# efirdc/Segmentation-Pipeline

Hardware: AMD Instinct MI355X
Metric: 3D patches/sec (128³, 4ch) train+infer at 1/2/4/8 MI355X; Dice vs CPU ref (higher is better)
Workload: dtype f32 (tensors, results and accumulation; the products of the 3x3x3 convolutions with >= 8 input channels run as six bf16 MFMAs on an EXACT three-way bf16 split of both f32 operands -- error vs f64 equal to the f32 MFMA kernels', profiles/r04_f32x3_accuracy.txt; the same step on v_mfma_f32_32x32x2_f32

## Files before the change

### include/m355seg.h

```cpp
#ifndef M355SEG_H
#define M355SEG_H

#include <stddef.h>
#include <stdint.h>

#ifdef __cplusplus
extern "C" {
#endif

#define M355_ABI_VERSION 3

enum {
  M355_OK = 0,
  M355_EINVALID_ARG = -1,
  M355_EUNSUPPORTED = -2,
  M355_ELAUNCH = -3,
  M355_EWORKSPACE = -4
};

enum { M355_F32 = 0 };

enum { M355_COMPUTE_F32 = 0, M355_COMPUTE_BF16 = 1, M355_COMPUTE_F16 = 2, M355_COMPUTE_F32X3 = 3 };

enum { M355_ACT_NONE = 0, M355_ACT_RELU = 1, M355_ACT_LEAKY_RELU = 2, M355_ACT_ELU = 3, M355_ACT_GELU = 4,
// ... 60 lines not shown
int m355_conv3d_bwd_data_h16(const m355_conv3d_desc* d, const void* dy16, int64_t dy16_batch_stride, const float* w,
                             float* dx, void* workspace, size_t workspace_bytes, void* stream);
size_t m355_conv3d_bwd_weight_h16_workspace(const m355_conv3d_desc* d);
int m355_conv3d_bwd_weight_h16(const m355_conv3d_desc* d, const void* x16, int64_t x16_batch_stride, const void* dy16,
                               int64_t dy16_batch_stride, const float* dy, float* dw, float* dbias, void* workspace,
                               size_t workspace_bytes, void* stream);

int m355_conv3d_plan(const m355_conv3d_desc* d, int32_t which, int32_t* out4);

int m355_conv3d_launch_plan(int32_t entry, const m355_conv3d_desc* d, const int64_t* batch_strides, const uint64_t* pointers,
                            size_t workspace_bytes, int64_t* out12);

size_t m355_conv3d_bwd_data_workspace(const m355_conv3d_desc* d);
int m355_conv3d_bwd_data(const m355_conv3d_desc* d, const float* dy, const float* w,
                         float* dx, void* workspace, size_t workspace_bytes, void* stream);

size_t m355_conv3d_bwd_weight_workspace(const m355_conv3d_desc* d);
int m355_conv3d_bwd_weight(const m355_conv3d_desc* d, const float* x, const float* dy,
                           float* dw, float* dbias,
                           void* workspace, size_t workspace_bytes, void* stream);

size_t m355_conv_transpose3d_workspace(const m355_conv3d_desc* d);
int m355_conv_transpose3d_fwd(const m355_conv3d_desc* d, const float* x, const float* w,
                              const float* bias, float* y,
                              void* workspace, size_t workspace_bytes, void* stream);
int m355_conv_transpose3d_bwd_data(const m355_conv3d_desc* d, const float* dy, const float* w,
                                   float* dx, void* workspace, size_t workspace_bytes,
                                   void* stream);
int m355_conv_transpose3d_bwd_weight(const m355_conv3d_desc* d, const float* x, const float* dy,
                                     float* dw, float* dbias,
                                     void* workspace, size_t workspace_bytes, void* stream);

int m355_conv_transpose3d_plan(const m355_conv3d_desc* d, int32_t which, const void* y_side, int32_t* out4);

int m355_conv_transpose3d_fwd_h16(const m355_conv3d_desc* d, const void* x16, int64_t x16_batch_stride,
                                  const float* w, const float* bias, void* y16, int64_t y16_batch_stride,
                                  int32_t compute, void* stream);

typedef struct m355_norm_desc {
  int32_t N, C;
  int64_t S;
  int32_t groups;
  int32_t act;
  float eps;
  float act_slope;
  int64_t x_batch_stride;
  int64_t y_batch_stride;
  int64_t add_batch_stride;
} m355_norm_desc;

int64_t m355_norm_num_stats(const m355_norm_desc* d);
size_t m355_norm_workspace(const m355_norm_desc* d);

int m355_norm_plan(const m355_norm_desc* d, int32_t which, int32_t* out4);

int m355_norm_stats(const m355_norm_desc* d, const float* x, float* mean, float* rstd,
                    float* running_mean, float* running_var, float momentum,
                    void* workspace, size_t workspace_bytes, void* stream);
int m355_norm_stats_from_partials(const m355_norm_desc* d, const float* stat_partials, int64_t slots,
                                  float* mean, float* rstd, float* running_mean, float* running_var,
                                  float momentum, void* workspace, size_t workspace_bytes, void* stream);
int m355_norm_stats_from_running(const m355_norm_desc* d, const float* running_mean,
                                 const float* running_var, float* mean, float* rstd,
                                 void* stream);
int m355_norm_act_fwd(const m355_norm_desc* d, const float* x, const float* mean,
                      const float* rstd, const float* gamma, const float* beta,
// ... 426 lines not shown
```

### segmentation-pipeline_amd/_lib.py

```python
import ctypes as C
import os

_HERE = os.path.dirname(os.path.abspath(__file__))
LIB_PATH = os.environ.get("M355_LIB_PATH") or os.path.join(_HERE, "libm355seg.so")

M355_OK = 0
ACT_NONE, ACT_RELU, ACT_LEAKY_RELU = 0, 1, 2
ACT_ELU, ACT_GELU, ACT_GELU_TANH, ACT_SILU = 3, 4, 5, 6
COMPUTE_F32, COMPUTE_BF16, COMPUTE_F16, COMPUTE_F32X3 = 0, 1, 2, 3
CONV_W_PACKED, CONV_SOFTMAX, CONV_SIGMOID = 1, 2, 4


class ConvDesc(C.Structure):
    _fields_ = [
        ("N", C.c_int32), ("Cin", C.c_int32), ("Cout", C.c_int32),
        ("D", C.c_int32), ("H", C.c_int32), ("W", C.c_int32),
        ("k", C.c_int32), ("stride", C.c_int32), ("pad", C.c_int32), ("out_pad", C.c_int32),
        ("x_batch_stride", C.c_int64), ("y_batch_stride", C.c_int64),
        ("compute", C.c_int32), ("flags", C.c_int32),
    ]


class PackItem(C.Structure):
    _fields_ = [("desc", ConvDesc), ("which", C.c_int32), ("w", C.c_void_p), ("packed", C.c_void_p)]


class NormDesc(C.Structure):
    _fields_ = [
        ("N", C.c_int32), ("C", C.c_int32), ("S", C.c_int64),
        ("groups", C.c_int32), ("act", C.c_int32),
        ("eps", C.c_float), ("act_slope", C.c_float),
        ("x_batch_stride", C.c_int64), ("y_batch_stride", C.c_int64), ("add_batch_stride", C.c_int64),
    ]


class AugStage(C.Structure):
    _fields_ = [("op", C.c_int32), ("order", C.c_int32), ("a", C.c_float), ("b", C.c_float), ("seed", C.c_uint64),
                ("stats", C.c_void_p), ("vec", C.c_void_p)]

# ... 112 lines not shown
    "m355_act16_pack_scaled": (C.c_int, [_P, _P, _i32, _i32, _i64, _i64, _i64, _i32, _f32, _P]),
    "m355_act16_unpack_scaled": (C.c_int, [_P, _P, _i32, _i32, _i64, _i64, _i64, _i32, _f32, _P]),
    "m355_conv3d_bwd_data_h16_c8": (C.c_int, [_CD, _P, _i64, _P, _P, _i64, _P, _sz, _P]),
    "m355_conv3d_bwd_weight_c8_workspace": (_sz, [_CD]),
    "m355_conv3d_bwd_weight_c8": (C.c_int, [_CD, _P, _i64, _P, _i64, _P, _P, _f32, _P, _sz, _P]),
    "m355_norm_act_bwd_c8": (C.c_int, [_ND, _P, _i64, _P, _i64, _P, _i64, _i32, _i32, _i32, _P, _P, _P, _P, _P, _i64, _P, _P,
                                       C.c_int, _f32, _i32, _P, _sz, _P]),
    "m355_norm_act_bwd_c8_reduce": (C.c_int, [_ND, _P, _i64, _P, _i64, _P, _i64, _i32, _i32, _i32, _P, _P, _P, _P, _P, _P,
                                              C.c_int, _P, _f32, _P, _i32, _P, _sz, _P]),
    "m355_norm_act_bwd_c8_apply": (C.c_int, [_ND, _P, _i64, _P, _i64, _P, _i64, _i32, _i32, _i32, _P, _P, _P, _P, _P, _P, _i64,
                                             _i32, _P]),
    "m355_avgpool3d_2x_bwd_h16": (C.c_int, [_P, _P, _P, _i32, _i32, _i32, _i32, _i32, _i64, _i64, _i64, _i32, _P]),
    "m355_upsample_trilinear2x_fwd_h16": (C.c_int, [_P, _P, _i32, _i32, _i32, _i32, _i32, _i64, _i64, _i32, _P]),
    "m355_upsample_trilinear2x_bwd_h16": (C.c_int, [_P, _P, _i32, _i32, _i32, _i32, _i32, _i64, _i64, _i32, _P]),
    "m355_act16_channel_scale": (C.c_int, [_P, _P, _P, _i32, _i32, _i64, _i64, _i64, _i32, _P]),
    "m355_space_to_depth2_h16": (C.c_int, [_P, _P, _i32, _i32, _i32, _i32, _i32, _i64, _i64, _i32, _P]),
    "m355_depth_to_space2_h16": (C.c_int, [_P, _P, _i32, _i32, _i32, _i32, _i32, _i64, _i64, _i32, _P]),
    "m355_conv_transpose3d_h16_bwd_supported": (_i32, [_CD]),
    "m355_conv_transpose3d_h16_bwd_workspace": (_sz, [_CD]),
    "m355_conv_transpose3d_bwd_data_h16": (C.c_int, [_CD, _P, _i64, _P, _P, _i64, _i32, _P]),
    "m355_conv_transpose3d_bwd_weight_h16": (C.c_int, [_CD, _P, _i64, _P, _i64, _P, _P, _f32, _i32, _P, _sz, _P]),
    "m355_conv3d_plan": (C.c_int, [_CD, _i32, C.POINTER(C.c_int32)]),
    "m355_conv3d_launch_plan": (C.c_int, [_i32, _CD, C.POINTER(_i64), C.POINTER(C.c_uint64), _sz, C.POINTER(_i64)]),
    "m355_conv3d_bwd_data_workspace": (_sz, [_CD]),
    "m355_conv3d_bwd_data": (C.c_int, [_CD, _P, _P, _P, _P, _sz, _P]),
    "m355_conv3d_bwd_weight_workspace": (_sz, [_CD]),
    "m355_conv3d_bwd_weight": (C.c_int, [_CD, _P, _P, _P, _P, _P, _sz, _P]),
    "m355_conv_transpose3d_workspace": (_sz, [_CD]),
    "m355_conv_transpose3d_plan": (C.c_int, [_CD, _i32, _P, C.POINTER(C.c_int32)]),
    "m355_conv_transpose3d_fwd": (C.c_int, [_CD, _P, _P, _P, _P, _P, _sz, _P]),
    "m355_conv_transpose3d_bwd_data": (C.c_int, [_CD, _P, _P, _P, _P, _sz, _P]),
    "m355_conv_transpose3d_bwd_weight": (C.c_int, [_CD, _P, _P, _P, _P, _P, _sz, _P]),
    "m355_conv_transpose3d_fwd_h16": (C.c_int, [_CD, _P, _i64, _P, _P, _P, _i64, _i32, _P]),
    "m355_norm_num_stats": (_i64, [_ND]),
    "m355_norm_workspace": (_sz, [_ND]),
    "m355_norm_plan": (C.c_int, [_ND, _i32, C.POINTER(C.c_int32)]),
    "m355_norm_stats": (C.c_int, [_ND, _P, _P, _P, _P, _P, _f32, _P, _sz, _P]),
    "m355_norm_stats_from_partials": (C.c_int, [_ND, _P, _i64, _P, _P, _P, _P, _f32, _P, _sz, _P]),
    "m355_norm_stats_from_running": (C.c_int, [_ND, _P, _P, _P, _P, _P]),
    "m355_norm_act_fwd": (C.c_int, [_ND, _P, _P, _P, _P, _P, _P, _P, _P]),
    "m355_norm_act_pool_fwd": (C.c_int, [_ND, _P, _P, _P, _P, _P, _P, _P, _i64, _i32, _i32, _i32, _P]),
    "m355_norm_act_bwd": (C.c_int, [_ND, _P, _P, _P, _P, _P, _P, _P, _P, _P, C.c_int, _P, _sz, _P]),
    "m355_norm_act_bwd_pool": (C.c_int, [_ND, _P, _P, _i64, _P, _i64, _i32, _i32, _i32, _P, _P, _P, _P, _P, _P, _P, C.c_int,
                                         _P, _sz, _P]),
    "m355_norm_sums": (C.c_int, [_ND, _P, _P, _i64, _P, _P, _sz, _P]),
    "m355_norm_stats_from_sums": (C.c_int, [_ND, _P, _P, _P, _P, _P, _f32, _P]),
    "m355_norm_act_bwd_reduce": (C.c_int, [_ND, _P, _P, _P, _P, _P, _P, _P, _P, C.c_int, _P, _P, _P, _sz, _P]),
    "m355_norm_act_bwd_apply": (C.c_int, [_ND, _P, _P, _P, _P, _P, _P, _P, _P, _P, _i64, _i32, _P]),
    "m355_norm_act_bwd_h16": (C.c_int, [_ND, _P, _P, _P, _P, _P, _P, _P, _P, _P, C.c_int, _P, _i64, _i32, _P, _sz, _P]),
    "m355_resample_plan": (C.c_int, [_i32, _i32, _i32, _i32, _i32, _i32, C.POINTER(_i64), C.POINTER(C.c_uint64), _i32,
                                     C.POINTER(_i64)]),
    "m355_avgpool3d_2x_fwd": (C.c_int, [_P, _P, _i32, _i32, _i32, _i32, _i32, _i64, _i64, _P]),
    "m355_avgpool3d_2x_bwd": (C.c_int, [_P, _P, _i32, _i32, _i32, _i32, _i32, _i64, _i64, _P]),
    "m355_avgpool3d_2x_bwd_add": (C.c_int, [_P, _P, _P, _i32, _i32, _i32, _i32, _i32, _i64, _i64, _i64, _P]),
    "m355_maxpool3d_2x_fwd": (C.c_int, [_P, _P, _P, _i32, _i32, _i32, _i32, _i32, _i64, _i64, _P]),
    "m355_maxpool3d_2x_bwd": (C.c_int, [_P, _P, _P, _P, _i32, _i32, _i32, _i32, _i32, _i64, _i64, _i64, _P]),
    "m355_maxpool3d_2x_fwd_h16": (C.c_int, [_P, _P, _P, _i32, _i32, _i32, _i32, _i32, _i64, _i64, _i32, _P]),
    "m355_maxpool3d_2x_bwd_h16": (C.c_int, [_P, _P, _P, _P, _i32, _i32, _i32, _i32, _i32, _i64, _i64, _i64, _i32, _P]),
    "m355_upsample_trilinear2x_fwd": (C.c_int, [_P, _P, _i32, _i32, _i32, _i32, _i32, _i64, _i64, _P]),
    "m355_upsample_trilinear2x_bwd": (C.c_int, [_P, _P, _i32, _i32, _i32, _i32, _i32, _i64, _i64, _P]),
    "m355_upsample_nearest2x_fwd": (C.c_int, [_P, _P, _i32, _i32, _i32, _i32, _i32, _i64, _i64, _P]),
    "m355_upsample_nearest2x_bwd": (C.c_int, [_P, _P, _i32, _i32, _i32, _i32, _i32, _i64, _i64, _P]),
    "m355_upsample_trilinear2x_hp_fwd": (C.c_int, [_P, _P, _i32, _i32, _i32, _i32, _i32, _i64, _i64, _P]),
    "m355_upsample_trilinear2x_hp_bwd": (C.c_int, [_P, _P, _i32, _i32, _i32, _i32, _i32, _i64, _i64, _P]),
    "m355_upsample_nearest2x_fwd_h16": (C.c_int, [_P, _P, _i32, _i32, _i32, _i32, _i32, _i64, _i64, _i32, _P]),
    "m355_upsample_nearest2x_bwd_h16": (C.c_int, [_P, _P, _i32, _i32, _i32, _i32, _i32, _i64, _i64, _i32, _P]),
# ... 185 lines not shown
```

### segmentation-pipeline_amd/csrc/abi.cpp

```cpp
#include "common.hpp"
#include <map>
#include <mutex>
#include <tuple>
#include <utility>

namespace m355 {
static thread_local char g_err[512] = "";
void set_error(const char* fmt, ...) {
  va_list ap;
  va_start(ap, fmt);
  vsnprintf(g_err, sizeof(g_err), fmt, ap);
  va_end(ap);
}

static int env_int(const char* name, int dflt) {
  const char* v = getenv(name);
  if (!v || !*v) return dflt;
  return atoi(v);
}
static Tuning read_tuning() {
  Tuning t;
  t.conv_ntw = env_int("M355_CONV_NTW", 0);
  t.conv_ksplit = env_int("M355_CONV_KSPLIT", 0);
  t.conv_slots = env_int("M355_CONV_SLOTS", 0);
  t.conv_persistent = env_int("M355_CONV_PERSISTENT", 1);
  t.no_small = env_int("M355_NO_SMALL", 0);
  t.smallcout_valu = env_int("M355_SMALLCOUT_VALU", 1);
  t.f32x3 = env_int("M355_F32X3", 1);
  t.f32x3_bww = env_int("M355_F32X3_BWW", 1);
  t.f32x3_edge = env_int("M355_F32X3_EDGE", 0);
  t.f32x3_convt = env_int("M355_F32X3_CONVT", 1);
  t.bww_nsplit = env_int("M355_BWW_NSPLIT", 0);
  t.bww_gen = env_int("M355_BWW_GEN", 2);
  t.bww_queue = env_int("M355_BWW_QUEUE", 1);
  t.h16_persistent = env_int("M355_H16_PERSISTENT", 1);
  t.tile16 = env_int("M355_TILE16", 1);
  t.convt_h16 = env_int("M355_CONVT_H16", 1);
  t.h16_w8 = env_int("M355_H16_W8", 1);
  t.h16_oneshot = env_int("M355_H16_ONESHOT", 1);
  t.h16_xcd = env_int("M355_H16_XCD", 1);
  t.conv_cube = env_int("M355_CONV_CUBE", 3);
  t.h16_order = env_int("M355_H16_ORDER", 3);
  t.fuse_softmax = env_int("M355_FUSE_SOFTMAX", 1);
  t.convt_wgs = env_int("M355_CONVT_WGS", 0);
  t.h16_stagger = env_int("M355_H16_STAGGER", 2);
  return t;
}
static Tuning g_tuning = read_tuning();
const Tuning& tuning() { return g_tuning; }

int num_cus() {
  static int cache[64] = {0};
  int dev = 0;
  if (hipGetDevice(&dev) != hipSuccess || dev < 0 || dev >= 64) {
    (void)hipGetLastError();
    return 256;
  }
  if (cache[dev] == 0) {
    int n = 0;
    if (hipDeviceGetAttribute(&n, hipDeviceAttributeMultiprocessorCount, dev) != hipSuccess || n <= 0) {
      (void)hipGetLastError();
      n = 256;
    }
    cache[dev] = n;
// ... 86 lines not shown
```

### segmentation-pipeline_amd/csrc/common.hpp

```cpp
#pragma once
#include <hip/hip_runtime.h>
#include <stdint.h>
#include <stdio.h>
#include <stdarg.h>
#include <stdlib.h>
#include <algorithm>
#include "../../include/m355seg.h"

namespace m355 {

void set_error(const char* fmt, ...);

static inline int64_t ceil_div(int64_t a, int64_t b) { return (a + b - 1) / b; }
static inline int64_t round_up(int64_t a, int64_t b) { return ceil_div(a, b) * b; }

static inline int check_launch(const char* what) {
  hipError_t e = hipGetLastError();
  if (e != hipSuccess) {
    set_error("%s: launch failed: %s", what, hipGetErrorString(e));
    return M355_ELAUNCH;
  }
  return M355_OK;
}

// ... 13 lines not shown
template <typename T>
__device__ __forceinline__ T wave_sum(T v) {
#pragma unroll
  for (int off = 32; off > 0; off >>= 1) v += __shfl_xor(v, off, 64);
  return v;
}

template <typename T, int NT, bool BCAST = false>
__device__ __forceinline__ T block_sum(T v, T* scratch) {
  v = wave_sum(v);
  const int lane = threadIdx.x & 63, w = threadIdx.x >> 6;
  __syncthreads();
  if (lane == 0) scratch[w] = v;
  __syncthreads();
  T r = T(0);
  if (BCAST || threadIdx.x == 0) {
#pragma unroll
    for (int i = 0; i < NT / 64; ++i) r += scratch[i];
  }
  return r;
}

__device__ __forceinline__ float sigmoid_f32(float v) { return 1.f / (1.f + expf(-v)); }

struct Tuning {
  int conv_ntw = 0, conv_ksplit = 0, conv_slots = 0, conv_persistent = 1;
  int no_small = 0, smallcout_valu = 1, bww_nsplit = 0, bww_gen = 2, bww_queue = 1, h16_persistent = 1, tile16 = 1, convt_h16 = 1, h16_w8 = 1, h16_oneshot = 1, h16_xcd = 1;
  int conv_cube = 3, h16_order = 3;
  int fuse_softmax = 1;
  int f32x3 = 1;
  int f32x3_bww = 1;
  int f32x3_edge = 0;
  int f32x3_convt = 1;
  int convt_wgs = 0;
  int h16_stagger = 2;
};
const Tuning& tuning();

static inline int64_t dense_or(int64_t stride, int64_t dense) { return stride ? stride : dense; }

int num_cus();

int* queue_state(hipStream_t st);
int* overflow_flag();

}
```

### segmentation-pipeline_amd/csrc/conv3d_common.hpp

```cpp
#pragma once
#include "common.hpp"
#include "h16.hpp"
#include "conv3d_route.hpp"

namespace m355 {


__device__ __forceinline__ int opaque(int v) {
  asm volatile("" : "+v"(v));
  return v;
}

__device__ __forceinline__ void queue_leave(int* __restrict__ counter) {
  if (threadIdx.x == 0) {
    if (atomicAdd(counter + 8, 1) == (int)gridDim.x - 1) {
#pragma unroll
      for (int r = 0; r < 9; ++r) counter[r] = 0;
    }
  }
}

template <int NTW, int GX>
struct FwdTile {
  static constexpr int GY = 32 / GX;
// ... 120 lines not shown
          s1[r] += t;
          s2[r] = fmaf(t, t, s2[r]);
        }
      }
      if (ok) {
#pragma unroll
        for (int r = 0; r < 4; ++r)
          if (ob + r < Cout) dst[base + (int64_t)r * DHW] = v[r];
      }
    }
  if (stat) {
#pragma unroll
    for (int r = 0; r < 4; ++r) {
#pragma unroll
      for (int off = 8; off >= 1; off >>= 1) {
        s1[r] += __shfl_xor(s1[r], off, 64);
        s2[r] += __shfl_xor(s2[r], off, 64);
      }
    }
    if ((lane & 15) == 0) {
#pragma unroll
      for (int r = 0; r < 4; ++r)
        if (ob + r < Cout) {
          stat[(int64_t)(ob + r) * 2] = s1[r];
          stat[(int64_t)(ob + r) * 2 + 1] = s2[r];
        }
    }
  }
}

int convt_fwd_x3_nvt(int Cin);
void launch_convt_fwd_x3(int nvt, dim3 grid, const float* x, const float* w, const float* bias, float* y, int Cin, int Cout,
                         int D, int H, int W, int64_t xbs, int64_t ybs, int mt_per_wg, hipStream_t st);

enum class ConvtKind {
  Direct,
  MfmaF32,
  X3,
  C8,
  H16,
  Unsupported
};
struct ConvtRoute {
  ConvtKind kind;
  int nvt;
  int mt;
  int mt_per_wg;
  int ks_n, ng;
  dim3 grid;
  size_t lds;
  int split, o_per_split;
  size_t slab_bytes;
  size_t dbias_offset, dbias_bytes;
  size_t workspace_bytes;
  int32_t plan_code[4];
};
ConvtRoute route_convt(const m355_conv3d_desc* d, int which, bool y_side_ok);
ConvtRoute route_convt_c8(const m355_conv3d_desc* d, int which);

struct ConvCall {
  const m355_conv3d_desc* d;
  const float* in;
  const void* in16;
  const float* w;
  const float* bias;
  const float* add;
// ... 86 lines not shown
```

### segmentation-pipeline_amd/csrc/conv3d_f32x3.hip

```cpp
#include "conv3d_common.hpp"

namespace m355 {

typedef __bf16 bf16x8 __attribute__((ext_vector_type(8)));
typedef unsigned u32x4 __attribute__((ext_vector_type(4)));

constexpr int X3_PAIRS = 14;
constexpr int X3_QUADS = 7;
__host__ __device__ constexpr int x3_pair_tap(int pair, int half) {
  return pair < 9 ? pair * 3 + half : (pair < 12 ? (pair - 9) * 9 + half * 3 + 2 : (pair == 12 ? half * 9 + 8 : 26));
}

__device__ __forceinline__ void x3_split(float v, unsigned& hi, unsigned& mid, unsigned& lo) {
  const unsigned u = __float_as_uint(v);
  hi = u & 0xffff0000u;
  const float r1 = (u & 0x7f800000u) == 0x7f800000u ? 0.f : v - __uint_as_float(hi);
  mid = __float_as_uint(r1) & 0xffff0000u;
  lo = __float_as_uint(r1 - __uint_as_float(mid));
}
__device__ __forceinline__ unsigned x3_pack(unsigned a, unsigned b) { return __builtin_amdgcn_perm(b, a, 0x07060302u); }

__device__ __forceinline__ void pack_w3_x3_item(const float* __restrict__ w, u32x4* __restrict__ wq, int64_t i, int Cout_w,
                                                int Cin_w, int kin, int mout, int nchunks, int transpose) {
  const int lane = (int)(i & 63);
// ... 1052 lines not shown
#pragma unroll
      for (int g = 0; g < NG; ++g) {
        if (v0 + g * 32 + l32 >= S) continue;
#pragma unroll
        for (int b = 0; b < 2; ++b)
          *reinterpret_cast<float2*>(yo + obase[g] + (int64_t)b * OW) =
              make_float2(acc[g][q * 4 + b * 2] + bv, acc[g][q * 4 + b * 2 + 1] + bv);
      }
    }
    mt += 4;
  }
}

int convt_fwd_x3_nvt(int Cin) {
  const int64_t cin2 = round_up(Cin, 16);
  for (int nvt : {128, 64, 32})
    if (cin2 * nvt * 6 <= 65536) return nvt;
  return 0;
}

void launch_convt_fwd_x3(int nvt, dim3 grid, const float* x, const float* w, const float* bias, float* y, int Cin, int Cout,
                         int D, int H, int W, int64_t xbs, int64_t ybs, int mt_per_wg, hipStream_t st) {
  const size_t lds = (size_t)round_up(Cin, 16) * nvt * 6;
#define M355_CONVT_X3(NVT) \
  hipLaunchKernelGGL(convt_k2s2_fwd_x3_kernel<NVT>, grid, dim3(256), lds, st, x, w, bias, y, Cin, Cout, D, H, W, xbs, ybs, mt_per_wg)
  switch (nvt) {
    case 128: M355_CONVT_X3(128); break;
    case 64: M355_CONVT_X3(64); break;
    default: M355_CONVT_X3(32); break;
  }
#undef M355_CONVT_X3
}

}
```

### segmentation-pipeline_amd/csrc/convt.hip

```cpp
#include "conv3d_common.hpp"

namespace m355 {

typedef float f32x16 __attribute__((ext_vector_type(16)));


template <int NVT>
__global__ __launch_bounds__(256) void convt_k2s2_fwd_mfma_kernel(
    const float* __restrict__ x, const float* __restrict__ w, const float* __restrict__ bias,
    float* __restrict__ y, int Cin, int Cout, int D, int H, int W, int64_t xbs, int64_t ybs, int mt_per_wg) {
  extern __shared__ float xs[];
  constexpr int NG = NVT / 32, P = 256 / NVT;
  const int tid = threadIdx.x, lane = tid & 63;
  const int wave = __builtin_amdgcn_readfirstlane(tid >> 6);
  const int half = lane >> 5, l32 = lane & 31;
  const int S = D * H * W;
  const int v0 = blockIdx.x * NVT;
  const int n = blockIdx.z;
  const float* xn = x + (int64_t)n * xbs;
  float* yn = y + (int64_t)n * ybs;
  constexpr int KC = 8;
  const int Cin2 = (Cin + 2 * KC - 1) / (2 * KC) * (2 * KC);
  const int OH = 2 * H, OW = 2 * W;
  const int64_t OS = (int64_t)S * 8;
// ... 1184 lines not shown
  if (compute == M355_COMPUTE_BF16) { M355_CONVT_FWD_T(__bf16) } else { M355_CONVT_FWD_T(_Float16) }
#undef M355_CONVT_FWD_T
#undef M355_CONVT_C8
#undef M355_CONVT_H16
}

static void launch_convt_bwd_data_h16(const ConvtRoute& r, const m355_conv3d_desc* d, const void* dy16, int64_t ybs,
                                      const float* w, void* dx16, int64_t xbs, int compute, hipStream_t st) {
  int* oflag = compute == M355_COMPUTE_F16 ? overflow_flag() : nullptr;
#define M355_CTBD(HT, MTW)                                                                                               \
  hipLaunchKernelGGL((convt_k2s2_bwd_data_h16_kernel<HT, MTW>), r.grid, dim3(256), r.lds, st, (const HT*)dy16, w,        \
                     (HT*)dx16, d->Cin, d->Cout, d->D, d->H, d->W, ybs, xbs, r.mt_per_wg, oflag)
#define M355_CTBD_T(HT)                                                  \
  if (r.mt_per_wg == 1) M355_CTBD(HT, 1); else if (r.mt_per_wg == 2) M355_CTBD(HT, 2); else M355_CTBD(HT, 4);
  if (compute == M355_COMPUTE_BF16) { M355_CTBD_T(__bf16) } else { M355_CTBD_T(_Float16) }
#undef M355_CTBD_T
#undef M355_CTBD
}

static void launch_convt_bww_c8(const ConvtRoute& r, const m355_conv3d_desc* d, const void* x16, int64_t xbs, const void* dy16,
                                int64_t ybs, float* dw, float grad_unscale, int compute, float* slab, hipStream_t st) {
#define M355_CTBW(HT, CT)                                                                                                 \
  hipLaunchKernelGGL((convt_k2s2_bww_c8_kernel<HT, CT>), r.grid, dim3(256), 0, st, (const HT*)x16, (const HT*)dy16, slab,  \
                     d->N, d->Cin, d->Cout, d->D, d->H, d->W, xbs, ybs, r.split, (int)r.grid.z)
#define M355_CTBW_T(HT) if (r.mt == 1) M355_CTBW(HT, 1); else if (r.mt == 2) M355_CTBW(HT, 2); else M355_CTBW(HT, 4);
  if (compute == M355_COMPUTE_BF16) { M355_CTBW_T(__bf16) } else { M355_CTBW_T(_Float16) }
#undef M355_CTBW_T
#undef M355_CTBW
  const int64_t total = (int64_t)d->Cin * d->Cout * 8;
  hipLaunchKernelGGL(convt_slab_reduce_t_kernel, dim3((unsigned)ceil_div(total, 64)), dim3(256), 0, st, slab, dw, d->Cin,
                     d->Cout, r.split, grad_unscale, overflow_flag());
}

}

using namespace m355;

extern "C" size_t m355_conv_transpose3d_workspace(const m355_conv3d_desc* d) {
  return d ? std::max(route_convt(d, 2, true).workspace_bytes, route_convt(d, 1, true).workspace_bytes) : 0;
}
extern "C" int32_t m355_conv_transpose3d_h16_bwd_supported(const m355_conv3d_desc* d) {
  return d && route_convt_c8(d, 1).kind != ConvtKind::Unsupported ? 1 : 0;
}
extern "C" size_t m355_conv_transpose3d_h16_bwd_workspace(const m355_conv3d_desc* d) {
  return d ? route_convt_c8(d, 2).workspace_bytes : 0;
}
extern "C" int m355_conv_transpose3d_plan(const m355_conv3d_desc* d, int32_t which, const void* y_side, int32_t* out4) {
  if (int rc = validate_convt(d, "conv_transpose3d_plan")) return rc;
  M355_REQUIRE(out4 && which >= 0 && which <= 5, M355_EINVALID_ARG, "conv_transpose3d_plan: null pointer or which not in 0..5");
  const ConvtRoute r = which < 3 ? route_convt(d, which, convt_y_side_ok(convt_geom(d), y_side)) : route_convt_c8(d, which - 3);
  std::copy_n(r.plan_code, 4, out4);
  return M355_OK;
}

extern "C" int m355_conv_transpose3d_fwd(const m355_conv3d_desc* d, const float* x, const float* w,
                                         const float* bias, float* y, void* workspace,
                                         size_t workspace_bytes, void* stream) {
  if (int rc = validate_convt(d, "conv_transpose3d_fwd")) return rc;
  M355_REQUIRE(x && w && y, M355_EINVALID_ARG, "conv_transpose3d_fwd: null pointer");
  (void)workspace; (void)workspace_bytes;
  hipStream_t st = (hipStream_t)stream;
  const ConvtGeom g = convt_geom(d);
  M355_REQUIRE(g.OD > 0 && g.OH > 0 && g.OW > 0, M355_EINVALID_ARG, "conv_transpose3d_fwd: empty output");
  const ConvtRoute r = route_convt(d, 0, convt_y_side_ok(g, y));
  switch (r.kind) {
    case ConvtKind::X3:
// ... 96 lines not shown
extern "C" int m355_conv_transpose3d_bwd_data_h16(const m355_conv3d_desc* d, const void* dy16, int64_t dy16_batch_stride,
                                                  const float* w, void* dx16, int64_t dx16_batch_stride, int32_t compute,
                                                  void* stream) {
  const char* who = "conv_transpose3d_bwd_data_h16";
  if (int rc = validate_convt(d, who)) return rc;
  const ConvtRoute r = route_convt_c8(d, 1);
  if (int rc = validate_convt_c8(who, d, r, dy16 && w && dx16, dx16, &dx16_batch_stride, dy16, &dy16_batch_stride, compute,
                                 0, CONVT_C8_BWD_UNSUPPORTED))
    return rc;
  launch_convt_bwd_data_h16(r, d, dy16, dy16_batch_stride, w, dx16, dx16_batch_stride, compute, (hipStream_t)stream);
  return check_launch("convt_k2s2_bwd_data_h16");
}

extern "C" int m355_conv_transpose3d_bwd_weight_h16(const m355_conv3d_desc* d, const void* x16, int64_t x16_batch_stride,
                                                    const void* dy16, int64_t dy16_batch_stride, float* dw, float* dbias,
                                                    float grad_unscale, int32_t compute, void* workspace,
                                                    size_t workspace_bytes, void* stream) {
  const char* who = "conv_transpose3d_bwd_weight_h16";
  if (int rc = validate_convt(d, who)) return rc;
  const ConvtRoute r = route_convt_c8(d, 2);
  if (int rc = validate_convt_c8(who, d, r, x16 && dy16 && dw && workspace, x16, &x16_batch_stride, dy16, &dy16_batch_stride,
                                 compute, workspace_bytes, CONVT_C8_BWD_UNSUPPORTED))
    return rc;
  hipStream_t st = (hipStream_t)stream;
  launch_convt_bww_c8(r, d, x16, x16_batch_stride, dy16, dy16_batch_stride, dw, grad_unscale, compute, (float*)workspace, st);
  if (dbias) {
    const int64_t OS = (int64_t)d->D * d->H * d->W * 8;
    if (int rc = launch_dbias_c8(dy16, dy16_batch_stride, dbias, d->N, d->Cout, OS, compute, grad_unscale,
                                 (char*)workspace + r.dbias_offset, st))
      return rc;
  }
  return check_launch("conv_transpose3d_bwd_weight_h16");
}
```

### segmentation-pipeline_amd/ops.py

```python
import ctypes as C
import os
import weakref
from dataclasses import dataclass
from typing import List, NamedTuple, Optional, Sequence

import numpy as np
import torch

from . import _lib
from ._lib import ACT_LEAKY_RELU, ACT_NONE, ACT_RELU, ConvDesc, NormDesc, check

FP32_SPLIT = os.environ.get("M355_FP32_SPLIT", "1") != "0"
_COMPUTE = {"fp32": _lib.COMPUTE_F32X3 if FP32_SPLIT else _lib.COMPUTE_F32, "fp32_mfma": _lib.COMPUTE_F32,
            "bf16": _lib.COMPUTE_BF16, "fp16": _lib.COMPUTE_F16}
_DT16 = {_lib.COMPUTE_BF16: torch.bfloat16, _lib.COMPUTE_F16: torch.float16}
_compute_mode = "fp32"


def set_precision(mode: str):
    global _compute_mode
    if mode not in _COMPUTE:
        raise ValueError(f"precision must be one of {sorted(_COMPUTE)}, not {mode!r}")
    _compute_mode = mode

# ... 1133 lines not shown
        x, xbs = _dense_channels(x)
        weight = weight.contiguous()
        N, Cin, D, H, W = x.shape
        Cout = weight.shape[1]
        od = lambda n: (n - 1) * stride - 2 * pad + k + out_pad
        oshape = (N, Cout, od(D), od(H), od(W))
        y = _alloc_out(out, oshape, x)
        y, ybs = _dense_channels(y)
        d = _conv_desc(N, Cin, Cout, D, H, W, k, stride, pad, xbs, ybs, out_pad, compute=_COMPUTE[_compute_mode])
        ws = _workspace(L.m355_conv_transpose3d_workspace(C.byref(d)), x.device)
        check(L.m355_conv_transpose3d_fwd(C.byref(d), _p(x), _p(weight), _p(bias), _p(y), _p(ws), ws.numel(),
                                          _stream()), "conv_transpose3d_fwd")
        ctx.desc, ctx.has_bias = d, bias is not None
        ctx.save_for_backward(x, weight)
        return y

    @staticmethod
    def backward(ctx, dy):
        L = _lib.lib()
        x, weight = ctx.saved_tensors
        d = ctx.desc
        dy, dybs = _dense_channels(dy)
        d = _conv_desc(d.N, d.Cin, d.Cout, d.D, d.H, d.W, d.k, d.stride, d.pad, d.x_batch_stride, dybs, d.out_pad, compute=d.compute)
        dx = dw = db = None
        if ctx.needs_input_grad[0]:
            dx = torch.empty((d.N, d.Cin, d.D, d.H, d.W), dtype=x.dtype, device=x.device)
            dd = _conv_desc(d.N, d.Cin, d.Cout, d.D, d.H, d.W, d.k, d.stride, d.pad, 0, dybs, d.out_pad, compute=d.compute)
            ws = _workspace(L.m355_conv_transpose3d_workspace(C.byref(dd)), x.device)
            check(L.m355_conv_transpose3d_bwd_data(C.byref(dd), _p(dy), _p(weight), _p(dx), _p(ws), ws.numel(),
                                                   _stream()), "conv_transpose3d_bwd_data")
        if ctx.needs_input_grad[1] or (ctx.has_bias and ctx.needs_input_grad[2]):
            dw = torch.empty_like(weight)
            db = torch.empty(d.Cout, dtype=weight.dtype, device=weight.device) if ctx.has_bias else None
            ws = _workspace(L.m355_conv_transpose3d_workspace(C.byref(d)), x.device)
            check(L.m355_conv_transpose3d_bwd_weight(C.byref(d), _p(x), _p(dy), _p(dw), _p(db), _p(ws),
                                                     ws.numel(), _stream()), "conv_transpose3d_bwd_weight")
        return dx, dw, db, None


def conv_transpose3d(x, weight, bias=None, stride=2, padding=0, output_padding=0, out: Optional[OutSlot] = None):
    k = weight.shape[2]
    if isinstance(x, Act16):
        if k == 2 and stride == 2 and padding == 0 and output_padding == 0:
            D, H, W = x.spatial
            y16 = _c8_out_slot(x, out, (2 * D, 2 * H, 2 * W), C=weight.shape[1])
            if torch.is_grad_enabled() and (_tracks_any(weight, bias) or x.requires_grad):
                return y16.with_t(_ConvTC8Fn.apply(x.t, weight, bias, x, y16))
            _convt_c8_fwd(x, weight.contiguous(), bias, y16)
            return y16
        y = _ConvT3dFn.apply(x.to_f32(), weight, bias, (k, stride, padding, output_padding, None))
        return _into_c8_slot(y, out, x.compute)
    return _ConvT3dFn.apply(x, weight, bias, (k, stride, padding, output_padding, out))


@dataclass
class NormCfg:
    groups: int
    eps: float
    act: int = ACT_NONE
    slope: float = 0.01
    training: bool = True
    momentum: float = 0.1
    running_mean: Optional[torch.Tensor] = None
    running_var: Optional[torch.Tensor] = None
    out: Optional[OutSlot] = None
    stats: Optional[dict] = None
    c8: int = 0
    dx_twin: int = 0
    twin: Optional["Act16"] = None
# ... 1648 lines not shown
```

Baseline: 50.25.

## Add bf16x3-split MFMA weight-gradient kernel for k2s2 transposed convolution

```diff
diff --git a/include/m355seg.h b/include/m355seg.h
--- a/include/m355seg.h
+++ b/include/m355seg.h
@@ -116,6 +116,14 @@
                                      void* workspace, size_t workspace_bytes, void* stream);
 
 int m355_conv_transpose3d_plan(const m355_conv3d_desc* d, int32_t which, const void* y_side, int32_t* out4);
+
+int32_t m355_conv_transpose3d_x3_bwd_supported(const m355_conv3d_desc* d, const void* y_side);
+size_t m355_conv_transpose3d_x3_bwd_workspace(const m355_conv3d_desc* d);
+int m355_conv_transpose3d_x3_bwd_plan(const m355_conv3d_desc* d, int32_t which, const void* y_side, int32_t* out4);
+int m355_conv_transpose3d_bwd_data_x3(const m355_conv3d_desc* d, const float* dy, const float* w, float* dx,
+                                      void* workspace, size_t workspace_bytes, void* stream);
+int m355_conv_transpose3d_bwd_weight_x3(const m355_conv3d_desc* d, const float* x, const float* dy, float* dw, float* dbias,
+                                        void* workspace, size_t workspace_bytes, void* stream);
 
 int m355_conv_transpose3d_fwd_h16(const m355_conv3d_desc* d, const void* x16, int64_t x16_batch_stride,
                                   const float* w, const float* bias, void* y16, int64_t y16_batch_stride,
diff --git a/segmentation-pipeline_amd/_lib.py b/segmentation-pipeline_amd/_lib.py
--- a/segmentation-pipeline_amd/_lib.py
+++ b/segmentation-pipeline_amd/_lib.py
@@ -5,6 +5,7 @@
 LIB_PATH = os.environ.get("M355_LIB_PATH") or os.path.join(_HERE, "libm355seg.so")
 
 M355_OK = 0
+M355_EUNSUPPORTED = -2
 ACT_NONE, ACT_RELU, ACT_LEAKY_RELU = 0, 1, 2
 ACT_ELU, ACT_GELU, ACT_GELU_TANH, ACT_SILU = 3, 4, 5, 6
 COMPUTE_F32, COMPUTE_BF16, COMPUTE_F16, COMPUTE_F32X3 = 0, 1, 2, 3
@@ -183,6 +184,11 @@
     "m355_conv_transpose3d_bwd_data": (C.c_int, [_CD, _P, _P, _P, _P, _sz, _P]),
     "m355_conv_transpose3d_bwd_weight": (C.c_int, [_CD, _P, _P, _P, _P, _P, _sz, _P]),
     "m355_conv_transpose3d_fwd_h16": (C.c_int, [_CD, _P, _i64, _P, _P, _P, _i64, _i32, _P]),
+    "m355_conv_transpose3d_x3_bwd_supported": (_i32, [_CD, _P]),
+    "m355_conv_transpose3d_x3_bwd_workspace": (_sz, [_CD]),
+    "m355_conv_transpose3d_x3_bwd_plan": (C.c_int, [_CD, _i32, _P, C.POINTER(C.c_int32)]),
+    "m355_conv_transpose3d_bwd_data_x3": (C.c_int, [_CD, _P, _P, _P, _P, _sz, _P]),
+    "m355_conv_transpose3d_bwd_weight_x3": (C.c_int, [_CD, _P, _P, _P, _P, _P, _sz, _P]),
     "m355_norm_num_stats": (_i64, [_ND]),
     "m355_norm_workspace": (_sz, [_ND]),
     "m355_norm_plan": (C.c_int, [_ND, _i32, C.POINTER(C.c_int32)]),
diff --git a/segmentation-pipeline_amd/csrc/abi.cpp b/segmentation-pipeline_amd/csrc/abi.cpp
--- a/segmentation-pipeline_amd/csrc/abi.cpp
+++ b/segmentation-pipeline_amd/csrc/abi.cpp
@@ -30,6 +30,7 @@
   t.f32x3_bww = env_int("M355_F32X3_BWW", 1);
   t.f32x3_edge = env_int("M355_F32X3_EDGE", 0);
   t.f32x3_convt = env_int("M355_F32X3_CONVT", 1);
+  t.f32x3_convt_bwd = env_int("M355_F32X3_CONVT_BWD", 1);
   t.bww_nsplit = env_int("M355_BWW_NSPLIT", 0);
   t.bww_gen = env_int("M355_BWW_GEN", 2);
   t.bww_queue = env_int("M355_BWW_QUEUE", 1);
diff --git a/segmentation-pipeline_amd/csrc/common.hpp b/segmentation-pipeline_amd/csrc/common.hpp
--- a/segmentation-pipeline_amd/csrc/common.hpp
+++ b/segmentation-pipeline_amd/csrc/common.hpp
@@ -69,6 +69,7 @@
   int f32x3_bww = 1;
   int f32x3_edge = 0;
   int f32x3_convt = 1;
+  int f32x3_convt_bwd = 1;
   int convt_wgs = 0;
   int h16_stagger = 2;
 };
diff --git a/segmentation-pipeline_amd/csrc/conv3d_common.hpp b/segmentation-pipeline_amd/csrc/conv3d_common.hpp
--- a/segmentation-pipeline_amd/csrc/conv3d_common.hpp
+++ b/segmentation-pipeline_amd/csrc/conv3d_common.hpp
@@ -176,6 +176,8 @@
 int convt_fwd_x3_nvt(int Cin);
 void launch_convt_fwd_x3(int nvt, dim3 grid, const float* x, const float* w, const float* bias, float* y, int Cin, int Cout,
                          int D, int H, int W, int64_t xbs, int64_t ybs, int mt_per_wg, hipStream_t st);
+void launch_convt_bww_x3(int mt, dim3 grid, const float* x, const float* dy, float* dw, float* dbias, float* slab, double* bslab,
+                         int N, int Cin, int Cout, int D, int H, int W, int64_t xbs, int64_t ybs, hipStream_t st);
 
 enum class ConvtKind {
   Direct,
diff --git a/segmentation-pipeline_amd/csrc/conv3d_f32x3.hip b/segmentation-pipeline_amd/csrc/conv3d_f32x3.hip
--- a/segmentation-pipeline_amd/csrc/conv3d_f32x3.hip
+++ b/segmentation-pipeline_amd/csrc/conv3d_f32x3.hip
@@ -1108,4 +1108,174 @@
 #undef M355_CONVT_X3
 }
 
-}
+template <int MT>
+__global__ __launch_bounds__(256, MT == 2 ? 3 : 2) void convt_k2s2_bwd_weight_x3_kernel(
+    const float* __restrict__ x, const float* __restrict__ dy, float* __restrict__ slab, double* __restrict__ bslab, int N,
+    int Cin, int Cout, int D, int H, int W, int64_t xbs, int64_t ybs, int nsplit) {
+  constexpr int NV = 32, CT = 32 * MT, RS = NV * 2 + 16, XJ = CT / 16;
+  __shared__ __attribute__((aligned(16))) unsigned char xs3[3 * CT * RS];
+  __shared__ __attribute__((aligned(16))) unsigned char dys3[3 * 128 * RS];
+  const int tid = threadIdx.x, lane = tid & 63;
+  const int wave = __builtin_amdgcn_readfirstlane(tid >> 6);
+  const int half = lane >> 5, l32 = lane & 31;
+  const int split = blockIdx.x, o0 = blockIdx.y * 16, c0 = blockIdx.z * CT;
+  const int S = D * H * W;
+  const int OH = 2 * H, OW = 2 * W;
+  const int64_t OS = (int64_t)S * 8;
+  const int64_t total = (int64_t)N * S;
+  const int64_t ntiles = (total + NV - 1) / NV;
+  const bool want_bias = bslab != nullptr && blockIdx.z == 0;
+
+  f32x16 acc[MT];
+#pragma unroll
+  for (int m = 0; m < MT; ++m)
+#pragma unroll
+    for (int r = 0; r < 16; ++r) acc[m][r] = 0.f;
+  float bsum[4] = {0.f, 0.f, 0.f, 0.f};
+
+  const int vp = tid & 15, part = tid >> 4, ab = part & 3, oq = part >> 2;
+  float2 xpf[XJ];
+  float4 dpf[4];
+  bool tok = false;
+  auto fetch = [&](int64_t tile) __attribute__((always_inline)) {
+    const int64_t g = tile * NV + 2 * vp;
+    tok = g < total;
+    const int64_t nn = tok ? g / S : 0;
+    const int v = tok ? (int)(g - nn * S) : 0;
+    const float* xp = x + nn * xbs + v;
+#pragma unroll
+    for (int j = 0; j < XJ; ++j) {
+      const int c = c0 + part + 16 * j;
+      xpf[j] = *reinterpret_cast<const float2*>(xp + ((tok && c < Cin) ? (int64_t)c * S : 0));
+    }
+    const float* dp = dy + nn * ybs + ((int64_t)(2 * (v / (W * H)) + (ab >> 1)) * OH + 2 * ((v / W) % H) + (ab & 1)) * OW +
+                      2 * (v % W);
+#pragma unroll
+    for (int j = 0; j < 4; ++j) {
+      const int o = o0 + oq + 4 * j;
+      dpf[j] = *reinterpret_cast<const float4*>(dp + ((tok && o < Cout) ? (int64_t)o * OS : 0));
+    }
+  };
+  auto put = [&](unsigned char* row, float a, float b, int plane_bytes) __attribute__((always_inline)) {
+    unsigned ha, ma, la, hb, mb, lb;
+    x3_split(a, ha, ma, la);
+    x3_split(b, hb, mb, lb);
+    *reinterpret_cast<unsigned*>(row) = x3_pack(ha, hb);
+    *reinterpret_cast<unsigned*>(row + plane_bytes) = x3_pack(ma, mb);
+    *reinterpret_cast<unsigned*>(row + 2 * plane_bytes) = x3_pack(la, lb);
+  };
+  auto commit = [&]() __attribute__((always_inline)) {
+#pragma unroll
+    for (int j = 0; j < XJ; ++j) {
+      const int c = part + 16 * j;
+      const bool ok = tok && c0 + c < Cin;
+      put(xs3 + c * RS + vp * 4, ok ? xpf[j].x : 0.f, ok ? xpf[j].y : 0.f, CT * RS);
+    }
+#pragma unroll
+    for (int j = 0; j < 4; ++j) {
+      const int ol = oq + 4 * j;
+      const bool ok = tok && o0 + ol < Cout;
+      const float4 q = ok ? dpf[j] : make_float4(0.f, 0.f, 0.f, 0.f);
+      unsigned char* row = dys3 + (ol * 8 + ab * 2) * RS + vp * 4;
+      put(row, q.x, q.z, 128 * RS);
+      put(row + RS, q.y, q.w, 128 * RS);
+      bsum[j] += (q.x + q.y) + (q.z + q.w);
+    }
+  };
+
+  if (split < ntiles) fetch(split);
+  for (int64_t tile = split; tile < ntiles; tile += nsplit) {
+    __syncthreads();
+    commit();
+    __syncthreads();
+    if (tile + nsplit < ntiles) fetch(tile + nsplit);
+    const unsigned char* xb = xs3 + l32 * RS + half * 16;
+    const unsigned char* db = dys3 + (wave * 32 + l32) * RS + half * 16;
+#pragma unroll
+    for (int s = 0; s < NV / 16; ++s) {
+      bf16x8 ah[MT], am[MT], al[MT];
+#pragma unroll
+      for (int m = 0; m < MT; ++m) {
+        ah[m] = *reinterpret_cast<const bf16x8*>(xb + (m * 32) * RS + s * 32);
+        am[m] = *reinterpret_cast<const bf16x8*>(xb + (CT + m * 32) * RS + s * 32);
+        al[m] = *reinterpret_cast<const bf16x8*>(xb + (2 * CT + m * 32) * RS + s * 32);
+      }
+      const bf16x8 bh = *reinterpret_cast<const bf16x8*>(db + s * 32);
+      const bf16x8 bm = *reinterpret_cast<const bf16x8*>(db + 128 * RS + s * 32);
+      const bf16x8 bl = *reinterpret_cast<const bf16x8*>(db + 2 * 128 * RS + s * 32);
+#pragma unroll
+      for (int m = 0; m < MT; ++m) acc[m] = __builtin_amdgcn_mfma_f32_32x32x16_bf16(al[m], bh, acc[m], 0, 0, 0);
+#pragma unroll
+      for (int m = 0; m < MT; ++m) acc[m] = __builtin_amdgcn_mfma_f32_32x32x16_bf16(am[m], bh, acc[m], 0, 0, 0);
+#pragma unroll
+      for (int m = 0; m < MT; ++m) acc[m] = __builtin_amdgcn_mfma_f32_32x32x16_bf16(ah[m], bh, acc[m], 0, 0, 0);
+#pragma unroll
+      for (int m = 0; m < MT; ++m) acc[m] = __builtin_amdgcn_mfma_f32_32x32x16_bf16(am[m], bm, acc[m], 0, 0, 0);
+#pragma unroll
+      for (int m = 0; m < MT; ++m) acc[m] = __builtin_amdgcn_mfma_f32_32x32x16_bf16(ah[m], bm, acc[m], 0, 0, 0);
+#pragma unroll
+      for (int m = 0; m < MT; ++m) acc[m] = __builtin_amdgcn_mfma_f32_32x32x16_bf16(ah[m], bl, acc[m], 0, 0, 0);
+    }
+  }
+  const int o = o0 + wave * 4 + (l32 >> 3);
+  if (o < Cout) {
+    float* sl = slab + (int64_t)split * Cin * Cout * 8;
+#pragma unroll
+    for (int m = 0; m < MT; ++m)
+#pragma unroll
+      for (int r = 0; r < 16; ++r) {
+        const int c = c0 + m * 32 + (r & 3) + 8 * (r >> 2) + 4 * half;
+        if (c < Cin) sl[((int64_t)c * Cout + o) * 8 + (l32 & 7)] = acc[m][r];
+      }
+  }
+  if (want_bias) {
+#pragma unroll
+    for (int j = 0; j < 4; ++j) {
+      const float s = wave_sum(bsum[j]);
+      const int ob = o0 + wave + 4 * j;
+      if (lane == 0 && ob < Cout) bslab[(int64_t)split * Cout + ob] = (double)s;
+    }
+  }
+}
+
+__global__ __launch_bounds__(256) void convt_k2s2_slab_reduce_x3_kernel(
+    const float* __restrict__ slab, float* __restrict__ out, int64_t total, int nsplit, const double* __restrict__ bslab,
+    float* __restrict__ dbias, int Cout, int eblocks) {
+  __shared__ double red[8][33];
+  const int e = threadIdx.x & 31, q = threadIdx.x >> 5;
+  const bool bias = (int)blockIdx.x >= eblocks;
+  const int64_t n = bias ? Cout : total;
+  const int64_t i = (int64_t)(bias ? blockIdx.x - eblocks : blockIdx.x) * 32 + e;
+  double v = 0.0;
+  if (i < n) {
+    if (bias) {
+      for (int s = q; s < nsplit; s += 8) v += bslab[(int64_t)s * n + i];
+    } else {
+#pragma unroll 4
+      for (int s = q; s < nsplit; s += 8) v += (double)slab[(int64_t)s * n + i];
+    }
+  }
+  red[q][e] = v;
+  __syncthreads();
+  if (q == 0 && i < n) {
+    const double r = ((red[0][e] + red[1][e]) + (red[2][e] + red[3][e])) + ((red[4][e] + red[5][e]) + (red[6][e] + red[7][e]));
+    (bias ? dbias : out)[i] = (float)r;
+  }
+}
+
+void launch_convt_bww_x3(int mt, dim3 grid, const float* x, const float* dy, float* dw, float* dbias, float* slab, double* bslab,
+                         int N, int Cin, int Cout, int D, int H, int W, int64_t xbs, int64_t ybs, hipStream_t st) {
+  const int nsplit = (int)grid.x;
+  if (mt == 2)
+    hipLaunchKernelGGL(convt_k2s2_bwd_weight_x3_kernel<2>, grid, dim3(256), 0, st, x, dy, slab, bslab, N, Cin, Cout, D, H, W,
+                       xbs, ybs, nsplit);
+  else
+    hipLaunchKernelGGL(convt_k2s2_bwd_weight_x3_kernel<4>, grid, dim3(256), 0, st, x, dy, slab, bslab, N, Cin, Cout, D, H, W,
+                       xbs, ybs, nsplit);
+  const int64_t total = (int64_t)Cin * Cout * 8;
+  const int eblocks = (int)ceil_div(total, 32), bblocks = dbias ? (int)ceil_div(Cout, 32) : 0;
+  hipLaunchKernelGGL(convt_k2s2_slab_reduce_x3_kernel, dim3((unsigned)(eblocks + bblocks)), dim3(256), 0, st, slab, dw, total,
+                     nsplit, bslab, dbias, Cout, eblocks);
+}
+
+}
diff --git a/segmentation-pipeline_amd/csrc/convt.hip b/segmentation-pipeline_amd/csrc/convt.hip
--- a/segmentation-pipeline_amd/csrc/convt.hip
+++ b/segmentation-pipeline_amd/csrc/convt.hip
@@ -1240,6 +1240,31 @@
                      d->Cout, r.split, grad_unscale, overflow_flag());
 }
 
+constexpr int64_t CONVT_X3_BWW_MIN_VOXELS = 512;
+static ConvtRoute route_convt_x3_bwd(const m355_conv3d_desc* d, int which, const void* dy) {
+  ConvtRoute r{};
+  r.kind = ConvtKind::Unsupported;
+  convt_plan_code(r, 0, 0, 0);
+  if (which != 2 || !convt_dims_ok(d) || !is_k2s2(d) || !convt_fits_i32(d)) return r;
+  if (d->compute != M355_COMPUTE_F32X3 || !tuning().f32x3 || !tuning().f32x3_convt_bwd) return r;
+  const ConvtGeom g = convt_geom(d);
+  if (d->W % 2 || g.ybs % 4 || g.xbs % 2 || ((uintptr_t)dy & 15)) return r;
+  const int64_t S = (int64_t)d->D * d->H * d->W;
+  if (d->N * S < CONVT_X3_BWW_MIN_VOXELS && tuning().f32x3_convt_bwd < 2) return r;
+  r.kind = ConvtKind::X3;
+  r.mt = d->Cin > 64 ? 4 : 2;
+  const int64_t otiles = ceil_div(d->Cout, 16), ctiles = ceil_div(d->Cin, 32 * r.mt);
+  const int64_t per_cu = r.mt == 2 ? 3 : 2;
+  r.split = (int)std::min(std::max<int64_t>(1, per_cu * num_cus() / (ctiles * otiles)), ceil_div(d->N * S, 32));
+  r.grid = dim3((unsigned)r.split, (unsigned)otiles, (unsigned)ctiles);
+  r.slab_bytes = (size_t)round_up((int64_t)r.split * d->Cin * d->Cout * 8 * 4, 256);
+  r.dbias_offset = r.slab_bytes;
+  r.dbias_bytes = (size_t)round_up((int64_t)r.split * d->Cout * 8, 256);
+  r.workspace_bytes = r.slab_bytes + r.dbias_bytes;
+  convt_plan_code(r, r.mt, r.split, 0);
+  return r;
+}
+
 }
 
 using namespace m355;
@@ -1402,3 +1427,49 @@
   }
   return check_launch("conv_transpose3d_bwd_weight_h16");
 }
+
+
+extern "C" int32_t m355_conv_transpose3d_x3_bwd_supported(const m355_conv3d_desc* d, const void* y_side) {
+  if (!d) return 0;
+  return (route_convt_x3_bwd(d, 1, y_side).kind == ConvtKind::X3 ? 1 : 0) | (route_convt_x3_bwd(d, 2, y_side).kind == ConvtKind::X3 ? 2 : 0);
+}
+extern "C" size_t m355_conv_transpose3d_x3_bwd_workspace(const m355_conv3d_desc* d) {
+  return d ? std::max(route_convt_x3_bwd(d, 1, nullptr).workspace_bytes, route_convt_x3_bwd(d, 2, nullptr).workspace_bytes) : 0;
+}
+extern "C" int m355_conv_transpose3d_x3_bwd_plan(const m355_conv3d_desc* d, int32_t which, const void* y_side, int32_t* out4) {
+  if (int rc = validate_convt(d, "conv_transpose3d_x3_bwd_plan")) return rc;
+  M355_REQUIRE(out4 && (which == 1 || which == 2), M355_EINVALID_ARG, "conv_transpose3d_x3_bwd_plan: null pointer or which not 1 | 2");
+  const ConvtRoute r = route_convt_x3_bwd(d, which, y_side);
+  std::copy_n(r.plan_code, 4, out4);
+  return M355_OK;
+}
+
+extern "C" int m355_conv_transpose3d_bwd_data_x3(const m355_conv3d_desc* d, const float* dy, const float* w, float* dx,
+                                                 void* workspace, size_t workspace_bytes, void* stream) {
+  const char* who = "conv_transpose3d_bwd_data_x3";
+  if (int rc = validate_convt(d, who)) return rc;
+  M355_REQUIRE(dy && w && dx, M355_EINVALID_ARG, "%s: null pointer", who);
+  (void)workspace; (void)workspace_bytes; (void)stream;
+  M355_REQUIRE(route_convt_x3_bwd(d, 1, dy).kind == ConvtKind::X3, M355_EUNSUPPORTED,
+               "%s: the data gradient has no split kernel (m355_conv_transpose3d_x3_bwd_supported bit 0): take "
+               "m355_conv_transpose3d_bwd_data", who);
+  return M355_EUNSUPPORTED;
+}
+
+extern "C" int m355_conv_transpose3d_bwd_weight_x3(const m355_conv3d_desc* d, const float* x, const float* dy, float* dw,
+                                                   float* dbias, void* workspace, size_t workspace_bytes, void* stream) {
+  const char* who = "conv_transpose3d_bwd_weight_x3";
+  if (int rc = validate_convt(d, who)) return rc;
+  M355_REQUIRE(x && dy && dw, M355_EINVALID_ARG, "%s: null pointer", who);
+  const ConvtRoute r = route_convt_x3_bwd(d, 2, dy);
+  M355_REQUIRE(r.kind == ConvtKind::X3 && ((uintptr_t)x & 7) == 0, M355_EUNSUPPORTED,
+               "%s: needs M355_COMPUTE_F32X3, kernel_size 2 / stride 2 / padding 0, even W, dy 16-byte and x 8-byte aligned, "
+               "batch strides that are multiples of 4 (dy) and 2 (x), and M355_F32X3_CONVT_BWD != 0 "
+               "(m355_conv_transpose3d_x3_bwd_supported bit 1): take m355_conv_transpose3d_bwd_weight", who);
+  M355_REQUIRE(workspace && workspace_bytes >= (dbias ? r.workspace_bytes : r.slab_bytes), M355_EWORKSPACE,
+               "%s: workspace too small (%zu < %zu)", who, workspace_bytes, dbias ? r.workspace_bytes : r.slab_bytes);
+  const ConvtGeom g = convt_geom(d);
+  launch_convt_bww_x3(r.mt, r.grid, x, dy, dw, dbias, (float*)workspace, dbias ? (double*)((char*)workspace + r.dbias_offset) : nullptr,
+                      d->N, d->Cin, d->Cout, d->D, d->H, d->W, g.xbs, g.ybs, (hipStream_t)stream);
+  return check_launch("convt_k2s2_bwd_weight_x3");
+}
diff --git a/segmentation-pipeline_amd/ops.py b/segmentation-pipeline_amd/ops.py
--- a/segmentation-pipeline_amd/ops.py
+++ b/segmentation-pipeline_amd/ops.py
@@ -1189,9 +1189,17 @@
         if ctx.needs_input_grad[1] or (ctx.has_bias and ctx.needs_input_grad[2]):
             dw = torch.empty_like(weight)
             db = torch.empty(d.Cout, dtype=weight.dtype, device=weight.device) if ctx.has_bias else None
-            ws = _workspace(L.m355_conv_transpose3d_workspace(C.byref(d)), x.device)
-            check(L.m355_conv_transpose3d_bwd_weight(C.byref(d), _p(x), _p(dy), _p(dw), _p(db), _p(ws),
-                                                     ws.numel(), _stream()), "conv_transpose3d_bwd_weight")
+            rc = _lib.M355_EUNSUPPORTED
+            if d.compute == _lib.COMPUTE_F32X3 and L.m355_conv_transpose3d_x3_bwd_supported(C.byref(d), _p(dy)) & 2:
+                ws = _workspace(L.m355_conv_transpose3d_x3_bwd_workspace(C.byref(d)), x.device)
+                rc = L.m355_conv_transpose3d_bwd_weight_x3(C.byref(d), _p(x), _p(dy), _p(dw), _p(db), _p(ws), ws.numel(),
+                                                           _stream())
+                if rc != _lib.M355_EUNSUPPORTED:
+                    check(rc, "conv_transpose3d_bwd_weight_x3")
+            if rc == _lib.M355_EUNSUPPORTED:
+                ws = _workspace(L.m355_conv_transpose3d_workspace(C.byref(d)), x.device)
+                check(L.m355_conv_transpose3d_bwd_weight(C.byref(d), _p(x), _p(dy), _p(dw), _p(db), _p(ws),
+                                                         ws.numel(), _stream()), "conv_transpose3d_bwd_weight")
         return dx, dw, db, None
 
 
```

After: 50.82, median of 6. +1.1%, better.
